# Keyteer/Mixed-precision_LU_Factorization

Hardware: AMD Instinct MI355X
Metric: LU GFLOP/s at N=32768 (1/2/4/8 GPUs); IR iterations to ||r||/||b||<1e-12 (higher is better)
Workload: dtype f64

## Files before the change

mixed-precision_lu_factorization_amd/csrc/factor_common.h:

```cpp
#pragma once
#include "mpf_internal.h"
#include <initializer_list>

struct FactorArgs {
    mpf_ctx *c; EvPool &ev; mpf_stats &st; const mpf_opts &o;
    double *d_A; int64_t lda, N; int32_t nb; int32_t *d_ipiv;
};
inline int pref_window_rows(const mpf_opts &o) { return o.trailing == MPF_TRAIL_FP64 ? HP_FP64_WINDOW_ROWS : 0; }
inline void stream_join(EvPool &ev, hipStream_t from, hipStream_t into) {
    hipEvent_t e = ev.get();
    hipEventRecord(e, from);
    hipStreamWaitEvent(into, e, 0);
}

int factor_check_args(mpf_ctx *c, const char *who, const char *ldname, int64_t N, int32_t nb, int64_t ld, const mpf_opts &o);
inline int wanted_superpanel(const mpf_ctx *c, const mpf_opts &o, int64_t N) {
    const bool f64 = o.trailing == MPF_TRAIL_FP64;
    int sb = f64 ? c->tune.superpanel_fp64 : c->tune.superpanel_fp16;
    if (!f64 && sb == 0) sb = (o.trailing == MPF_TRAIL_FP16 && N >= 24576) ? 6 : 4;
    return o.superpanel > 0 ? (o.superpanel > 8 ? 8 : o.superpanel) : sb;
}
int factor_report(mpf_ctx *c, mpf_stats &st, int rc, const std::function<hipError_t()> &wait, const char *what, const char *timeout_text);

struct PanelView {
    double *A; int64_t lda;
    int64_t k; int pr, pc;
    MovedList *ml; int32_t *ipiv;
};
int panel_pivots(const FactorArgs &f, const PanelView &v, hipStream_t s, int waiters, bool generic = false);
int panel_tail(const FactorArgs &f, const PanelView &v, hipStream_t s);
int panel_pieces(const FactorArgs &f, const PanelView &v, int np, const std::function<int(int)> &after_piece = nullptr);
int panel_chain(const FactorArgs &f, int64_t k, hipStream_t s);
struct ChainEnd { int rc = 0; hipEvent_t a = nullptr, b = nullptr; };
ChainEnd chain_behind(const FactorArgs &f, int64_t nx, hipEvent_t e1);
int factor_epilogue(const FactorArgs &f, int rc, bool sink, int sb, bool side_streams);

int launch_generic_update(mpf_ctx *c, const mpf_opts &o, int64_t m, int64_t n, int pc, const double *L21, int64_t ldl, double *U12, int64_t ldu);
inline int launch_inner_u_image(mpf_ctx *c, const mpf_opts &o, const double *U12, int64_t ldu, int pc, int64_t n, int64_t inner_u_off) {
    return launch_cvt_u12(c, U12, ldu, pc, n, o.trailing == MPF_TRAIL_FP16X3, inner_u_off);
}
inline int launch_inner_gemm(mpf_ctx *c, const mpf_opts &o, int64_t m, int64_t n, int pc, const double *L21, int64_t ldl, double *U12, int64_t ldu, int64_t inner_u_off) {
    if (o.trailing == MPF_TRAIL_FP64) return launch_dgemm_minus(c, m, n, pc, L21, ldl, U12, ldu, U12 + pc, ldu);
    return launch_hgemm_images(c, m, n, pc, U12 + pc, ldu, false, o.trailing == MPF_TRAIL_FP16X3, 0, 0, inner_u_off);
}

struct FarView {
    double *A; int64_t lda;
    float *W; int64_t ldw, ncols;
    const double *Lsp; int64_t ldl;
    const double *L11; int64_t ld11;
};
struct ImageGeom { int kst; int64_t inner_u_off, brow_l_off; };
inline ImageGeom image_geom(int64_t N, int64_t far_cap, int sb, int nb, int h_kmax, bool f64) {
    const int kst = (int)(((int64_t)sb * nb + 63) & ~(int64_t)63);
    return {kst, (!f64 && far_cap > 0) ? far_cap * kst : 0, N * h_kmax};
}
int far_zero_padding(const FactorArgs &f, int64_t ncols, const ImageGeom &g);
int far_block_row(const FactorArgs &f, const FarView &v, const ImageGeom &g, int64_t s0, int p);
int far_big_update(const FactorArgs &f, const FarView &v, const ImageGeom &g, int64_t s0, int64_t s1, int64_t col, int64_t ncols, int img);

struct RmView {
    double *A; int64_t lda;
    double *R; int64_t ldr;
    double *a(int64_t i, int64_t j) const { return A + j * lda + i; }
    double *r(int64_t i, int64_t j) const { return R + i * ldr + j; }
};
int rm_swap(const FactorArgs &f, const RmView &v, hipStream_t s, int64_t c, int64_t w, std::initializer_list<const MovedList *> lists, int64_t scratch_off);
int rm_solve_u(const FactorArgs &f, const RmView &v, hipStream_t s, const double *L11, int64_t ld11, int64_t k, int pc, int64_t c, int64_t w);
int rm_update(const FactorArgs &f, const RmView &v, hipStream_t s, int64_t ku, int K, int64_t r0, int64_t rows, int64_t c, int64_t w, const double *Limg, int64_t ldimg);
int rm_home(const FactorArgs &f, const RmView &v, hipStream_t s, int64_t row, int64_t rows, int64_t c, int64_t w, int64_t split = 0);
int rm_l_image(const FactorArgs &f, hipStream_t s, const double *src, int64_t lds, int64_t rows, int64_t cols, double *img, int64_t ldimg);
bool pivots_fit_beside_update(const mpf_ctx *c, int64_t rows);
int factor_lookahead_rm(mpf_ctx *c, double *d_A, int64_t lda, int64_t N, int32_t nb, int32_t *d_ipiv, const mpf_opts &o, mpf_stats &st, bool pairs);
```

mixed-precision_lu_factorization_amd/csrc/factor_rm.cpp:

```cpp
#include "factor_common.h"
#include <cstdio>

int rm_swap(const FactorArgs &f, const RmView &v, hipStream_t s, int64_t c, int64_t w, std::initializer_list<const MovedList *> lists, int64_t scratch_off) {
    return f.ev.timed(f.st.ms_laswp, s, [&] {
        int e = 0;
        for (const MovedList *ml : lists) if (!e) e = launch_laswp_from_list_rm64(f.c, v.r(0, c), v.ldr, w, ml, scratch_off);
        return e; });
}
int rm_solve_u(const FactorArgs &f, const RmView &v, hipStream_t s, const double *L11, int64_t ld11, int64_t k, int pc, int64_t c, int64_t w) {
    return f.ev.timed(f.st.ms_trsm, s, [&] { return launch_dtrsm_llnu_strided(f.c, pc, w, L11, ld11, v.r(k, c), v.ldr, 1); });
}
int rm_update(const FactorArgs &f, const RmView &v, hipStream_t s, int64_t ku, int K, int64_t r0, int64_t rows, int64_t c, int64_t w, const double *Limg, int64_t ldimg) {
    const int e = f.ev.timed(f.st.ms_gemm, s, [&] { return launch_dgemm_minus(f.c, w, rows, K, v.r(ku, c), v.ldr, Limg, ldimg, v.r(r0, c), v.ldr); });
    count_gemm(f.st, f.o, rows, w, K);
    return e;
}
int rm_home(const FactorArgs &f, const RmView &v, hipStream_t s, int64_t row, int64_t rows, int64_t c, int64_t w, int64_t split) {
    return f.ev.timed(f.st.ms_cvt, s, [&] {
        if (split <= 0) return launch_transpose64(f.c, v.a(row, c), v.lda, v.r(row, c), v.ldr, rows, w, false);
        int e = launch_transpose64(f.c, v.a(row, c), v.lda, v.r(row, c), v.ldr, split, w, false);
        if (!e) e = launch_transpose64(f.c, v.a(row + split, c), v.lda, v.r(row + split, c), v.ldr, rows - split, w, false);
        return e; });
}
int rm_l_image(const FactorArgs &f, hipStream_t s, const double *src, int64_t lds, int64_t rows, int64_t cols, double *img, int64_t ldimg) {
// ... 281 lines not shown
}

static int rm_turn_one_lane(const FactorArgs &f, const RmView &v, RmLoop &L, const RmTurn &t) {
    mpf_ctx *c = f.c; EvPool &ev = f.ev; hipStream_t S = c->stream, P = c->pstream, T = c->tstream;
    const int64_t N = f.N, k = t.k, nx = t.nx, n = t.n, ce = L.ce; const int pc = t.pc, pc2 = t.pc2;
    const double *L11 = v.a(k, k);
    const int64_t cw = ce - nx - pc2;
    int rc = 0;
    if (L.was_two) {
        stream_join(ev, T, S);
        if (L.chain_a) hipStreamWaitEvent(S, L.chain_a, 0);
        if (L.chain_b) hipStreamWaitEvent(S, L.chain_b, 0);
        L.was_two = false;
    }
    hipEvent_t lt_ready = ev.get();
    {
        stream_join(ev, S, P);
        StreamSwap sw(c, P);
        rc = rm_l_image(f, P, v.a(nx, k), v.lda, n, pc, t.LT, pc);
        hipEventRecord(lt_ready, P);
    }
    if (!rc) rc = rm_swap(f, v, S, nx, ce - nx, {t.lk}, 0);
    if (!rc) rc = rm_solve_u(f, v, S, L11, v.lda, k, pc, nx, t.ns);
    hipStreamWaitEvent(S, lt_ready, 0);
    if (!rc) rc = rm_update(f, v, S, k, pc, nx, n, nx, t.ns, t.LT, pc);
    if (rc) return rc;
    if (!t.has_next)
        return rm_home(f, v, S, k, N - k, nx, N - nx, pc);
    rc = rm_home(f, v, S, nx, N - nx, nx, pc2);
    if (rc) return rc;
    hipEvent_t e1 = ev.get();
    hipEventRecord(e1, S);
    const ChainEnd next = chain_behind(f, nx, e1);
    rc = next.rc;
    if (rc) return rc;
    if (cw > 0) rc = rm_solve_u(f, v, S, L11, v.lda, k, pc, nx + pc2, cw);
    if (rc) return rc;
    hipStream_t H = T ? T : S;
    {
        if (T) stream_join(ev, S, T);
        StreamSwap sw(c, H);
        rc = rm_home(f, v, H, k, pc, nx, ce - nx);
        if (L.sink && !rc && ce == N) sink_notify(c, (int)(k / f.nb) + 1, H);
    }
    if (!rc && cw > 0) rc = rm_update(f, v, S, k, pc, nx, n, nx + pc2, cw, t.LT, pc);
    if (rc) return rc;
    L.chain_a = next.a; L.chain_b = next.b;
    hipStreamWaitEvent(S, L.chain_a, 0);
    if (L.chain_b) hipStreamWaitEvent(S, L.chain_b, 0);
    if (f.o.verbose) printf("panel k=%lld rows=%lld cols=%d (look-ahead, row-major copy)\n", (long long)nx, (long long)(N - nx), pc2);
    return 0;
}

int factor_lookahead_rm(mpf_ctx *c, double *d_A, int64_t lda, int64_t N, int32_t nb, int32_t *d_ipiv, const mpf_opts &o, mpf_stats &st, bool pairs) {
    hipStream_t S = c->stream, P = c->pstream, T = c->tstream;
    EvPool ev(c);
    ev.keep = &st.ms_gemm;
    const FactorArgs f{c, ev, st, o, d_A, lda, N, nb, d_ipiv};
    const RmView v{d_A, lda, c->r64, N};
    int rc = 0;
    RmLoop L;
    L.sink = sink_take(c, d_A, lda, N, nb);
    L.lp = (c->late && !c->late->taken && c->late->nseg > 0 && lda == N) ? c->late : nullptr;
    if (L.lp) L.lp->taken = true;
    L.ce = L.lp ? L.lp->c0[0] : N;
    { hipEvent_t e = ev.get(); hipEventRecord(e, S); hipStreamWaitEvent(P, e, 0); if (T) hipStreamWaitEvent(T, e, 0); }
    const int pc0 = (int)(N < nb ? N : nb);
    if (N > 1) {
        hipEvent_t e0 = ev.get();
        {
            StreamSwap sw(c, P);
            rc = ev.timed(st.ms_hpanel, P, [&] {
                int e = launch_hgetf2(c, d_A, lda, nullptr, 0, (int)N, pc0, 0, d_ipiv, nullptr, 0, c->lists, 0, pref_window_rows(o));
                if (!e) e = launch_laswp_from_list(c, d_A, lda, pc0, c->lists);
                if (!e) e = launch_dgetf2_npv(c, d_A, lda, (int)N, pc0, o.fused_panel, 0);
                return e; });
            hipEventRecord(e0, P);
        }
        st.panels++;
        if (!rc && pc0 < L.ce) rc = rm_l_image(f, S, v.a(0, pc0), lda, N, L.ce - pc0, v.r(0, pc0), v.ldr);
        hipStreamWaitEvent(S, e0, 0);
        L.chain_a = e0;
    }
    L.init_done = ev.get();
    hipEventRecord(L.init_done, S);
    if (pairs && !rc && !L.sink && !L.lp && T && N > 1) rc = factor_rm_pairs(f, v, L);
    for (int64_t k = L.k0; k < N && rc == 0; k += nb) {
        const RmTurn t(f, k);
        if (N - k <= 1 || t.nx >= N) break;
        rc = rm_replay_late(f, v, L, t);
        if (rc) break;
        const int64_t cw = L.ce - t.nx - t.pc2;
        const bool want_two = T && c->tune.fp64_two_lanes > 0 && t.has_next && pivots_fit_beside_update(c, N - t.nx) &&
                              (N - t.nx) > c->tune.chain_pipeline_below && cw >= c->tune.fp64_two_lanes;
        if (!want_two) L.cm = -1;
        const bool resplit = want_two && lane_split(c, t.nx + t.pc2, L.ce, L.cm);
        if (L.cm >= 0) rc = rm_turn_two_lanes(f, v, L, t, resplit);
        else {
            rc = rm_turn_one_lane(f, v, L, t);
            if (!t.has_next) break;
        }
    }
    if (!rc && L.lp && L.lseg < L.lp->nseg) rc = fail(c, -1, "factor_lookahead_rm: a late column segment was never brought up to date (plan beyond the matrix)");
    if (T) stream_join(ev, T, S);
    stream_join(ev, P, S);
    return factor_epilogue(f, rc, L.sink, 1, true);
}
```

mixed-precision_lu_factorization_amd/csrc/laswp.hip:

```cpp
#include "mpf_internal.h"

constexpr int LASWP_CPB = 16;

__global__ __launch_bounds__(256) void laswp_plan_kernel(const int *ipiv, int k, int cols, MovedList *out) {
    __shared__ int slot[HP_MAXCOLS];
    __shared__ int rowof[2 * HP_MAXCOLS];
    __shared__ int content[2 * HP_MAXCOLS];
    __shared__ int used[2 * HP_MAXCOLS];
    __shared__ int count;
    const int t = threadIdx.x;
    for (int s = t; s < 2 * cols; s += 256) { content[s] = s; used[s] = s < cols; rowof[s] = s < cols ? k + s : -1; }
    if (t == 0) count = 0;
    __syncthreads();
    if (t < cols) {
        const int p = ipiv[t] - 1;
        int s;
        if (p < k + cols) s = p - k;
        else {
            int first = t;
            for (int i = 0; i < t; ++i)
                if (ipiv[i] - 1 == p) { first = i; break; }
            s = cols + first;
            if (first == t) { rowof[s] = p; used[s] = 1; }
        }
// ... 338 lines not shown
__global__ __launch_bounds__(256) void lazy_gather_kernel(const double *__restrict__ A, long long lda, long long n, long long r0,
                                                         int w, const int *__restrict__ G, long long g0, double *__restrict__ T, long long ldt) {
    const long long d = r0 + (long long)blockIdx.x * 256 + threadIdx.x;
    if (d >= n) return;
    const long long sr = G[d - g0];
    const int c0 = blockIdx.y * 16;
#pragma unroll 8
    for (int c = c0; c < c0 + 16 && c < w; ++c) T[(d - r0) + (long long)c * ldt] = A[sr + (long long)c * lda];
}
__global__ __launch_bounds__(256) void lazy_scatter_kernel(const double *__restrict__ A, long long lda, long long n, long long r0,
                                                          int w, const int *__restrict__ F, double *__restrict__ T, long long ldt) {
    const long long r = r0 + (long long)blockIdx.x * 256 + threadIdx.x;
    if (r >= n) return;
    const long long d = (long long)F[r] - r0;
    const int c0 = blockIdx.y * 16;
#pragma unroll 4
    for (int c = c0; c < c0 + 16 && c < w; ++c) T[d + (long long)c * ldt] = A[r + (long long)c * lda];
}
__global__ __launch_bounds__(256) void lazy_copyback_kernel(double *__restrict__ A, long long lda, long long n, long long r0, int w,
                                                           const double *__restrict__ T, long long ldt) {
    const long long r = r0 + (long long)blockIdx.x * 256 + threadIdx.x;
    if (r >= n) return;
    const int c0 = blockIdx.y * 16;
#pragma unroll 4
    for (int c = c0; c < c0 + 16 && c < w; ++c) A[r + (long long)c * lda] = T[(r - r0) + (long long)c * ldt];
}

constexpr int LAZY1_THREADS = 1024;
constexpr int LAZY1_SLOTS = 32;
__host__ __device__ inline long long lazy_snap_offset(long long n, long long step, long long q) {
    return (q - 1) * n - step * ((q - 1) * q / 2);
}
__global__ __launch_bounds__(LAZY1_THREADS) void lazy_map_all_kernel(int *F, int *G, long long n, int nb, int npanels, int sb,
                                                                    const MovedList *lists, int *snap) {
    const int t = threadIdx.x;
    for (long long i = t; i < n; i += LAZY1_THREADS) { F[i] = (int)i; G[i] = (int)i; }
    __syncthreads();
    for (int p = npanels - 1; p >= 1; --p) {
        const MovedList *ml = lists + p;
        int m = ml->n;
        if (m > LASWP_MAXMOVED) m = LASWP_MAXMOVED;
        int v = 0, s = 0;
        if (t < m) { v = F[ml->dst[t]]; s = ml->src[t]; }
        __syncthreads();
        if (t < m) { F[s] = v; G[v] = s; }
        __syncthreads();
        if (p % sb) continue;
        const long long r0 = (long long)p * nb;
        int *sq = snap + lazy_snap_offset(n, (long long)sb * nb, p / sb);
        for (long long d = r0 + t; d < n; d += LAZY1_THREADS) sq[d - r0] = G[d];
    }
}
constexpr int LAZY1_LDS_ROWS = 16384;
template <int SLOTS>
__global__ __launch_bounds__(LAZY1_THREADS) void lazy_apply_all_kernel(double *A, long long lda, long long n, int nb, int sb, int b0,
                                                                      const int *snap) {
    constexpr int H = SLOTS * LAZY1_THREADS < LAZY1_LDS_ROWS ? SLOTS * LAZY1_THREADS : LAZY1_LDS_ROWS;
    constexpr int PASSES = SLOTS * LAZY1_THREADS / H;
    __shared__ double seg[H];
    const int b = b0 + (int)(blockIdx.x / (unsigned)nb);
    const long long q = b / sb + 1;
    const long long r0 = q * sb * nb;
    const int rows = (int)(n - r0);
    const int *Gq = snap + lazy_snap_offset(n, (long long)sb * nb, q);
    double *col = A + ((long long)b * nb + (long long)(blockIdx.x % (unsigned)nb)) * lda + r0;
    const int t = threadIdx.x;
    double v[SLOTS];
    constexpr int GRP = SLOTS < 8 ? SLOTS : 8;
#pragma unroll
    for (int pass = 0; pass < PASSES; ++pass) {
        const int base = pass * H;
        if (pass > 0) __syncthreads();
#pragma unroll
        for (int j0 = 0; j0 < H / LAZY1_THREADS; j0 += GRP) {
            double x[GRP];
#pragma unroll
            for (int j = 0; j < GRP; ++j) {
                const int r = base + (j0 + j) * LAZY1_THREADS + t;
                x[j] = col[(unsigned)(r < rows ? r : rows - 1) & (unsigned)(SLOTS * LAZY1_THREADS - 1)];
            }
#pragma unroll
            for (int j = 0; j < GRP; ++j) seg[(j0 + j) * LAZY1_THREADS + t] = x[j];
            asm volatile("" ::: "memory");
        }
        __syncthreads();
#pragma unroll
        for (int i0 = 0; i0 < SLOTS; i0 += GRP) {
            int rel[GRP];
            double x[GRP];
#pragma unroll
            for (int i = 0; i < GRP; ++i) {
                const int d = (i0 + i) * LAZY1_THREADS + t;
                rel[i] = Gq[(unsigned)(d < rows ? d : rows - 1) & (unsigned)(SLOTS * LAZY1_THREADS - 1)] - (int)r0 - base;
            }
#pragma unroll
            for (int i = 0; i < GRP; ++i) {
                x[i] = seg[(unsigned)rel[i] < (unsigned)H ? rel[i] : 0];
                asm volatile("" : "+v"(x[i]));
            }
#pragma unroll
            for (int i = 0; i < GRP; ++i)
                if (PASSES == 1 || (unsigned)rel[i] < (unsigned)H) v[i0 + i] = x[i];
            asm volatile("" ::: "memory");
        }
    }
    __syncthreads();
#pragma unroll
    for (int i = 0; i < SLOTS; ++i) {
        const int d = i * LAZY1_THREADS + t;
        if (d < rows) col[(unsigned)d & (unsigned)(SLOTS * LAZY1_THREADS - 1)] = v[i];
    }
}
template <int SLOTS>
static void lazy_apply_launch(mpf_ctx *c, double *A, int64_t lda, int64_t N, int nb, int sb, int b0, int nblocks, const int *snap) {
    lazy_apply_all_kernel<SLOTS><<<(unsigned)((int64_t)nblocks * nb), LAZY1_THREADS, 0, c->stream>>>(A, lda, N, nb, sb, b0, snap);
}
int64_t lazy_snap_elems(int64_t N, int nb, int npanels, int sb) {
    if (sb < 1) sb = 1;
    return npanels < 2 ? 0 : lazy_snap_offset(N, (int64_t)sb * nb, (npanels - 1) / sb + 1);
}
static int launch_lazy_left_swaps_onepass(mpf_ctx *c, double *A, int64_t lda, int64_t N, int nb, int npanels, const MovedList *lists, int sb) {
    const int64_t step = (int64_t)sb * nb;
    const int Q = (npanels - 1) / sb;
    c->lazy_onepass_blocks = 0;
    if (Q < 1) return 0;
    const int64_t need = lazy_snap_elems(N, nb, npanels, sb);
    if (c->lazy_snap.cap() < need) {
        MPF_HIP_TRY(c, hipStreamSynchronize(c->stream));
        MPF_HIP_TRY(c, c->lazy_snap.grow(need));
    }
    int *snap = c->lazy_snap;
    lazy_map_all_kernel<<<1, LAZY1_THREADS, 0, c->stream>>>(c->Fmap, c->Fmap + N, N, nb, npanels, sb, lists, snap);
    int64_t cap = c->tune.lazy_onepass_max_rows;
    if (cap > (int64_t)LAZY1_THREADS * LAZY1_SLOTS) cap = (int64_t)LAZY1_THREADS * LAZY1_SLOTS;
    const int nblk = Q * sb;
    int b1 = nblk;
    for (int b = 0; b < nblk; ++b) {
        const int64_t q = b / sb + 1, r0 = q * step, rows = N - r0;
        if (rows <= cap) { b1 = b; break; }
        dim3 grid((unsigned)((rows + 255) / 256), (unsigned)((nb + 15) / 16));
        double *Ab = A + (int64_t)b * nb * lda;
        lazy_gather_kernel<<<grid, 256, 0, c->stream>>>(Ab, lda, N, r0, nb, snap + lazy_snap_offset(N, step, q), r0, c->perm_tmp, rows);
        lazy_copyback_kernel<<<grid, 256, 0, c->stream>>>(Ab, lda, N, r0, nb, c->perm_tmp, rows);
    }
    for (int b = b1; b < nblk;) {
        const int64_t rows = N - (b / sb + 1) * step;
        int slots = 2;
        while ((int64_t)LAZY1_THREADS * slots < rows) slots *= 2;
        int e = b + 1;
        while (e < nblk && (N - (e / sb + 1) * step) * 2 > (int64_t)LAZY1_THREADS * slots) ++e;
        if (slots == 2) e = nblk;
        switch (slots) {
        case 32: lazy_apply_launch<32>(c, A, lda, N, nb, sb, b, e - b, snap); break;
        case 16: lazy_apply_launch<16>(c, A, lda, N, nb, sb, b, e - b, snap); break;
        case 8: lazy_apply_launch<8>(c, A, lda, N, nb, sb, b, e - b, snap); break;
        case 4: lazy_apply_launch<4>(c, A, lda, N, nb, sb, b, e - b, snap); break;
        default: lazy_apply_launch<2>(c, A, lda, N, nb, sb, b, e - b, snap); break;
        }
        b = e;
    }
    c->lazy_onepass_blocks = nblk - b1;
    MPF_HIP_TRY(c, hipGetLastError());
    return 0;
// ... 31 lines not shown
```

mixed-precision_lu_factorization_amd/csrc/mpf_factor.cpp:

```cpp
#include "factor_common.h"
#include <climits>
#include <cstdio>

int factor_check_args(mpf_ctx *c, const char *who, const char *ldname, int64_t N, int32_t nb, int64_t ld, const mpf_opts &o) {
    const std::string w = std::string(who) + ": ";
    if (N <= 0 || nb <= 0) return fail(c, -1, w + "N and panel width must be positive");
    if (ld < N) return fail(c, -1, w + ldname + " < N");
    if (N > INT_MAX / 2) return fail(c, -1, w + "N too large");
    if (nb > 65535) return fail(c, -1, w + "panel width > 65535");
    if (o.trailing < MPF_TRAIL_FP64 || o.trailing > MPF_TRAIL_FP16X3) return fail(c, -1, w + "unknown trailing mode");
    return 0;
}

int factor_report(mpf_ctx *c, mpf_stats &st, int rc, const std::function<hipError_t()> &wait, const char *what, const char *timeout_text) {
    hipEventRecord(c->ev1, c->stream);
    const hipError_t se = wait();
    if (rc) return rc;
    if (se != hipSuccess) return fail(c, -2, std::string(what) + " failed: " + hipGetErrorString(se));
    float ms = 0;
    hipEventElapsedTime(&ms, c->ev0, c->ev1);
    st.ms_total = ms;
    int info = 0, flags0 = 0;
    MPF_HIP_TRY(c, hipMemcpy(&info, &c->ws->info, sizeof(int), hipMemcpyDeviceToHost));
    MPF_HIP_TRY(c, hipMemcpy(&flags0, &c->ws->hp_timeouts, sizeof(int), hipMemcpyDeviceToHost));
// ... 213 lines not shown
    return e;
}

ChainEnd chain_behind(const FactorArgs &f, int64_t nx, hipEvent_t e1) {
    mpf_ctx *c = f.c; EvPool &ev = f.ev;
    const PanelView v = panel_at(f, nx);
    hipStream_t P = c->pstream, T = c->tstream;
    const int np = dgetf2_npv_pieces(c, v.pc);
    const int waiters = (c->tune.gate_wait_value && c->hp_signal) ? 0 : laswp_gated_grid(v.pc);
    const bool piped = c->tune.chain_pipeline && np != 0 && T && P &&
        !(f.o.trailing == MPF_TRAIL_FP64 && v.pr > c->tune.chain_pipeline_below) &&
        hgetf2_fits_beside(c, v.pr, v.pc, waiters);
    ChainEnd r;
    hipStreamWaitEvent(P, e1, 0);
    if (!piped) {
        r.rc = panel_chain(f, nx, P);
        r.a = ev.get();
        hipEventRecord(r.a, P);
        return r;
    }
    hipStreamWaitEvent(T, e1, 0);
    {
        StreamSwap sw(c, P);
        r.rc = panel_pivots(f, v, P, waiters);
        r.a = ev.get();
        hipEventRecord(r.a, P);
    }
    if (!r.rc) {
        StreamSwap sw(c, T);
        r.rc = ev.timed(f.st.ms_dpanel, T, [&] { return panel_pieces(f, v, np); });
        r.b = ev.get();
        hipEventRecord(r.b, T);
    }
    f.st.panels++;
    return r;
}

int factor_epilogue(const FactorArgs &f, int rc, bool sink, int sb, bool side_streams) {
    mpf_ctx *c = f.c;
    hipStream_t S = c->stream;
    const int npanels = (int)((f.N + f.nb - 1) / f.nb);
    if (sink) sink_notify(c, npanels, S);
    else if (!rc) {
        rc = f.ev.timed(f.st.ms_laswp, S, [&] { return launch_lazy_left_swaps(c, f.d_A, f.lda, f.N, f.nb, npanels, c->lists, sb); });
        f.st.lazy_onepass_blocks = c->lazy_onepass_blocks;
    }
    hipError_t se = sink_stream_wait(c, S);
    hipError_t sp = side_streams ? sink_stream_wait(c, c->pstream) : hipSuccess;
    if (side_streams && c->tstream) { const hipError_t stt = sink_stream_wait(c, c->tstream); if (sp == hipSuccess) sp = stt; }
    if (!rc && (se != hipSuccess || sp != hipSuccess))
        return fail(c, -2, std::string("factorization failed: ") + hipGetErrorString(se != hipSuccess ? se : sp));
    f.ev.collect();
    f.st.lookahead = side_streams ? 1 : 0;
    return rc;
}

static int factor_lookahead(mpf_ctx *c, double *d_A, int64_t lda, int64_t N, int32_t nb, int32_t *d_ipiv,
                            const mpf_opts &o, mpf_stats &st) {
    hipStream_t S = c->stream, P = c->pstream;
    EvPool ev(c);
    ev.keep = &st.ms_gemm;
    const FactorArgs f{c, ev, st, o, d_A, lda, N, nb, d_ipiv};
    int rc = 0;
    const bool sink = sink_take(c, d_A, lda, N, nb);
    stream_join(ev, S, P);
    {
        const int pc = (int)(N < nb ? N : nb), pr = (int)N;
        if (pr > 1) {
            rc = ev.timed(st.ms_hpanel, S, [&] {
                int e = launch_hgetf2(c, d_A, lda, nullptr, 0, pr, pc, 0, d_ipiv, nullptr, 0, c->lists, 0, pref_window_rows(o));
                const int64_t first = (int64_t)pc + nb < N ? (int64_t)pc + nb : N;
                if (!e) e = launch_laswp_from_list(c, d_A, lda, first, c->lists);
                if (!e) e = launch_dgetf2_npv(c, d_A, lda, pr, pc, o.fused_panel, 0);
                return e;
            });
            st.panels++;
        }
    }
    for (int64_t k = 0; k < N && rc == 0; k += nb) {
        const int pc = (int)((N - k) < nb ? (N - k) : nb);
        if (N - k <= 1 || k + pc >= N) break;
        const int64_t n = N - k - pc;
        const int64_t nx = k + pc;
        const int pc2 = (int)((N - nx) < nb ? (N - nx) : nb);
        const bool has_next = (N - nx) > 1;
        double *Ap = d_A + k * lda + k;
        double *A12 = d_A + nx * lda + k;
        const int64_t ns = has_next ? pc2 : n;
        rc = ev.timed(st.ms_trsm, S, [&] { return launch_dtrsm_llnu(c, pc, ns, Ap, lda, A12, lda); });
        if (rc) break;
        rc = ev.timed(st.ms_gemm, S, [&] {
            int e = o.trailing != MPF_TRAIL_FP64 ? launch_cvt_l21(c, Ap + pc, lda, n, pc, o.trailing == MPF_TRAIL_FP16X3) : 0;
            if (!e) e = trail_gemm(c, o, n, ns, pc, Ap + pc, A12, A12 + pc, lda);
            return e; });
        if (rc) break;
        count_gemm(st, o, n, ns, pc);
        if (!has_next) break;
        hipEvent_t e1 = ev.get();
        hipEventRecord(e1, S);
        const ChainEnd next = chain_behind(f, nx, e1);
        rc = next.rc;
        if (rc) break;
        if (n > pc2) {
            rc = ev.timed(st.ms_laswp, S, [&] {
                return launch_laswp_from_list(c, d_A + (nx + pc2) * lda, lda, N - nx - pc2, c->lists + (k / nb)); });
            if (rc) break;
            double *A12r = A12 + (int64_t)pc2 * lda;
            rc = ev.timed(st.ms_trsm, S, [&] { return launch_dtrsm_llnu(c, pc, n - pc2, Ap, lda, A12r, lda); });
            if (rc) break;
            if (sink) sink_notify(c, (int)(k / nb) + 1, S);
            rc = ev.timed(st.ms_gemm, S, [&] { return trail_gemm(c, o, n, n - pc2, pc, Ap + pc, A12r, A12r + pc, lda); });
            if (rc) break;
            count_gemm(st, o, n, n - pc2, pc);
        }
        hipStreamWaitEvent(S, next.a, 0);
        if (next.b) hipStreamWaitEvent(S, next.b, 0);
        rc = ev.timed(st.ms_laswp, S, [&] {
            const int64_t s0 = nx + pc2;
            const int64_t sw = (N - s0) < nb ? (N - s0) : nb;
            return sw > 0 ? launch_laswp_from_list(c, d_A + s0 * lda, lda, sw, c->lists + (nx / nb)) : 0;
        });
        if (o.verbose) printf("panel k=%lld rows=%lld cols=%d (look-ahead)\n", (long long)nx, (long long)(N - nx), pc2);
    }
    if (sink) stream_join(ev, P, S);
    return factor_epilogue(f, rc, sink, 1, true);
}

static int factor_superpanel(mpf_ctx *c, double *d_A, int64_t lda, int64_t N, int32_t nb, int32_t *d_ipiv, const mpf_opts &o,
                             mpf_stats &st, int sb, bool overlap) {
    hipStream_t S = c->stream, P = overlap ? c->pstream : c->stream;
    hipStream_t Ci = (overlap && c->tstream) ? c->tstream : c->stream;
    const bool lanes = Ci != S;
    EvPool ev(c);
    ev.keep = &st.ms_gemm;
    const FactorArgs f{c, ev, st, o, d_A, lda, N, nb, d_ipiv};
    int rc = 0;
    const bool split = o.trailing == MPF_TRAIL_FP16X3;
    const bool f64 = o.trailing == MPF_TRAIL_FP64;
    const bool use32 = !f64 && c->tune.fp16_work32 != 0 && N > (int64_t)(sb + 1) * nb;
    float *W = nullptr;
    const int64_t ldw = N;
    if (use32) {
        MPF_HIP_TRY(c, c->w32.grow(N * N));
        W = c->w32;
    }
    if (overlap) stream_join(ev, S, P);
    const int64_t sbw = (int64_t)sb * nb;
    const ImageGeom g = image_geom(N, N - (int64_t)(sb + 1) * nb, sb, nb, c->h_kmax, f64);
    auto width = [&](int64_t k) { return (int)((N - k) < nb ? (N - k) : nb); };
    auto side_chain = [&](int64_t kx, hipEvent_t e1, hipEvent_t &e2) -> int {
        if (!overlap) return panel_chain(f, kx, S);
        const ChainEnd next = chain_behind(f, kx, e1);
        e2 = next.a;
        if (!next.rc && next.b) {
            e2 = ev.get();
            hipStreamWaitEvent(c->tstream, next.a, 0);
            hipEventRecord(e2, c->tstream);
        }
        return next.rc;
    };
    hipEvent_t img_ready = nullptr;
    auto l21_image = [&](int64_t k, int pc) -> int {
        if (f64) return 0;
        const int64_t mrows = N - k - pc;
        if (mrows <= 0) return 0;
        hipStream_t Is = (lanes && P != S) ? P : Ci;
        if (Is != Ci) stream_join(ev, Ci, Is);
        StreamSwap sw(c, Is);
        int e = ev.timed(st.ms_cvt, Is, [&] { return launch_cvt_l21(c, d_A + k * lda + k + pc, lda, mrows, pc, split); });
        if (Is != Ci) { img_ready = ev.get(); hipEventRecord(img_ready, Is); } else img_ready = nullptr;
        return e;
    };
    auto inner_step = [&](int64_t k, int pc, int64_t col0, int64_t ncols, bool first) -> int {
        if (ncols <= 0) return 0;
        StreamSwap sw(c, Ci);
        double *Ap = d_A + k * lda + k, *A12 = d_A + col0 * lda + k;
// ... 167 lines not shown
```

mixed-precision_lu_factorization_amd/csrc/mpf_host.cpp:

```cpp
#include "mpf_internal.h"
#include <climits>
#include <cstdio>
#include <cstdlib>
#include <cstring>

std::string &noctx_error() { static thread_local std::string s; return s; }

namespace {
struct OptDesc { const char *name, *env; size_t off; bool wide; long long lo, hi; };
#define OPT_I(field, env, lo, hi) {#field, env, offsetof(MpfTuning, field), false, lo, hi}
#define OPT_L(field, env, lo, hi) {#field, env, offsetof(MpfTuning, field), true, lo, hi}
const OptDesc kOpts[] = {
    OPT_I(safe_pivots, "MPF_SAFE_PIVOTS", 0, 1),
    OPT_I(pivot_fp64, "MPF_PIVOT_FP64", 0, 2),
    OPT_I(chain_pipeline, "MPF_CHAIN_PIPELINE", 0, 1),
    OPT_L(chain_pipeline_below, "MPF_CHAIN_PIPELINE_BELOW", 0, 1ll << 40),
    OPT_I(fp16_work32, "MPF_FP16_WORK32", 0, 1),
    OPT_I(superpanel_fp16, "MPF_SUPERPANEL", 0, 8),
    OPT_I(superpanel_fp64, "MPF_SUPERPANEL_FP64", 1, 8),
    OPT_I(no_lookahead, "MPF_NO_LOOKAHEAD", 0, 1),
    OPT_I(verbose, "MPF_VERBOSE", 0, 1),
    OPT_I(timeline, "MPF_TIMELINE", 0, 1),
    OPT_L(hp_spin_limit, "MPF_HP_SPIN_LIMIT", 1, 1ll << 31),
    OPT_L(hp_gate_ticks, "MPF_HP_GATE_TICKS", 0, 1ll << 40),
    OPT_I(hp_acq_fence, "MPF_HP_ACQ_FENCE", 0, 1),
    OPT_I(hp_window, "MPF_HP_WINDOW", -1, 1 << 30),
    OPT_I(hgemm_pad, "MPF_HGEMM_PAD", 0, 65536),
    OPT_I(hgemm_split_pad, "MPF_HGEMM_SPLIT_PAD", 0, 65536),
    OPT_I(hgemm_big, "MPF_HGEMM_BIG", 0, 1),
    OPT_I(hgemm_big_tile, "MPF_HGEMM_BIG_TILE", 0, 5),
    OPT_I(hgemm_mfma16, "MPF_HGEMM_MFMA16", 0, 1),
    OPT_I(dgemm_dma, "MPF_DGEMM_DMA", 0, 1),
    OPT_I(lazy_gather, "MPF_LAZY_GATHER", 0, 2),
    OPT_I(lazy_onepass_max_rows, "MPF_LAZY_ONEPASS_MAX_ROWS", 0, 32768),
    OPT_I(dpanel_fused_form, "MPF_DPANEL_FUSED", 0, 1),
    OPT_I(dist_instalments, "MPF_DIST_INSTALMENTS", 0, 1),
    OPT_L(dist_instalment_min_bytes, "MPF_DIST_INSTALMENT_MIN_BYTES", 0, 1ll << 40),
    OPT_I(generic_fused, "MPF_GENERIC_FUSED", 0, 1),
    OPT_I(fp16_fused, "MPF_FP16_FUSED", 0, 1),
    OPT_I(fp64_rowmajor, "MPF_FP64_ROWMAJOR", 0, 1),
    OPT_L(fp64_rowmajor_min_n, "MPF_FP64_ROWMAJOR_MIN_N", 0, 1ll << 40),
    OPT_I(trsm_laswp_fused, "MPF_TRSM_LASWP_FUSED", 0, 1),
    OPT_I(fp64_two_lanes, "MPF_FP64_TWO_LANES", 0, 1 << 30),
    OPT_I(fp64_lane_a_pct, "MPF_FP64_LANE_A_PCT", 20, 90),
    OPT_I(fp64_pair, "MPF_FP64_PAIR", 0, 1),
    OPT_L(fp64_pair_min_n, "MPF_FP64_PAIR_MIN_N", 0, 1ll << 40),
    OPT_I(event_timers, "MPF_EVENT_TIMERS", 0, 2),
    OPT_I(dist_world1_loop, "MPF_DIST_WORLD1_LOOP", 0, 1),
    OPT_I(gesv_fp64_tflops, "MPF_GESV_FP64_TFLOPS", 0, 1000),
    OPT_I(gate_wait_value, "MPF_GATE_WAIT_VALUE", 0, 1),
    OPT_I(host_sink, "MPF_HOST_SINK", 0, 1),
    OPT_I(sink_trace, "MPF_SINK_TRACE", 0, 1),
    OPT_I(hp_half_slabs, "MPF_HP_HALF_SLABS", 0, 1),
    OPT_I(hp_half_slabs_rows, "MPF_HP_HALF_SLABS_ROWS", 256, 32768),
    OPT_I(hp_local_xcd, "MPF_HP_LOCAL_XCD", 0, 2),
    OPT_I(host_late_parts, "MPF_HOST_LATE_PARTS", 0, 4),
    OPT_L(host_late_min_n, "MPF_HOST_LATE_MIN_N", 0, 1ll << 40),
    OPT_I(host_first_pct, "MPF_HOST_FIRST_PCT", 5, 100),
    OPT_I(host_late_q_pct, "MPF_HOST_LATE_Q_PCT", 1, 1000),
    OPT_L(host_sink_min_n, "MPF_HOST_SINK_MIN_N", 0, 1ll << 40),
    OPT_I(dist_solve_p2p, "MPF_DIST_SOLVE_P2P", 0, 1),
    OPT_I(gmres_group_tiles, "MPF_GMRES_GROUP_TILES", 0, 16),
#ifdef MPF_PROBE
    OPT_I(hp_stamp, "MPF_HP_STAMP", 0, 1),
    OPT_I(hp_r256_upto, "MPF_HP_R256_UPTO", 0, 1 << 30),
    OPT_I(dgemm_w8, "MPF_DGEMM_W8", 0, 1),
    OPT_I(gemm_lds_pad, "MPF_GEMM_LDS_PAD", 0, 65536),
    OPT_I(hgemm_big_reg, "MPF_HGEMM_BIG_REG", 0, 1),
    OPT_I(hgemm_dbg, "MPF_HGEMM_DBG", 0, 8191),
#endif
};
#undef OPT_I
#undef OPT_L
void opt_store(MpfTuning &t, const OptDesc &d, long long v) {
    if (v < d.lo) v = d.lo;
    if (v > d.hi) v = d.hi;
    char *p = (char *)&t + d.off;
    if (d.wide) *(long long *)p = v; else *(int *)p = (int)v;
}
long long opt_load(const MpfTuning &t, const OptDesc &d) {
    const char *p = (const char *)&t + d.off;
    return d.wide ? *(const long long *)p : (long long)*(const int *)p;
}
void tuning_from_env(MpfTuning &t) {
    for (const OptDesc &d : kOpts)
        if (const char *e = getenv(d.env)) if (*e) opt_store(t, d, atoll(e));
}
}

extern "C" {

int mpf_create(mpf_ctx **out, int device) {
    if (!out) return -1;
    *out = nullptr;
// ... 295 lines not shown
```

mixed-precision_lu_factorization_amd/csrc/mpf_internal.h:

```cpp
#pragma once
#include <hip/hip_runtime.h>
#include <stdint.h>
#include <string>
#include <vector>
#include <functional>
#include "../../include/mpf_c.h"

constexpr int HP_R = 256;
constexpr int HP_T = 512;
constexpr int HP_MAXG = 256;
constexpr int HP_MAXCOLS = 256;
constexpr int LASWP_MAXMOVED = 2 * HP_MAXCOLS;

struct MovedList {
    int n;
    int pad[3];
    int src[LASWP_MAXMOVED];
    int dst[LASWP_MAXMOVED];
};

struct MpfWorkspace {
    unsigned long long cand[2][HP_MAXG];
    int flags[16];
    unsigned long long rowbuf[2][HP_MAXG][HP_MAXCOLS / 2];
    int hp_timeouts;
    int pad0[3];
    MovedList list0;
    int info;
    int pad[3];
    unsigned long long hp_stamps[8];
    unsigned long long hp_progress;
    unsigned long long hp_xcd_target;
    unsigned long long hp_xcd_roles;
};

struct MpfTuning {
    int safe_pivots = 0;
    int pivot_fp64 = 0;
    int chain_pipeline = 1;
    long long chain_pipeline_below = 10240;
    int fp16_work32 = 1;
    int superpanel_fp16 = 0;
    int superpanel_fp64 = 1;
    int no_lookahead = 0;
    int verbose = 0;
    int timeline = 0;
    long long hp_spin_limit = 1ll << 21;
    long long hp_gate_ticks = 200000000ll;
    int hp_window = -1;
    int hp_acq_fence = 0;
    int hgemm_pad = 0;
    int hgemm_split_pad = 32768;
    int hgemm_big = 1;
    int hgemm_mfma16 = 1;
    int hgemm_big_tile = 0;
    int dgemm_dma = 1;
    int lazy_gather = 2;
    int lazy_onepass_max_rows = 32768;
    int dpanel_fused_form = 1;
    int dist_instalments = 1;
    long long dist_instalment_min_bytes = 8ll << 20;
    int fp16_fused = 0;
    int generic_fused = 1;
    int fp64_rowmajor = 1;
    long long fp64_rowmajor_min_n = 8192;
    int trsm_laswp_fused = 1;
    int fp64_two_lanes = 8192;
    int dist_solve_p2p = 0;
    int host_sink = 1;
    int hp_local_xcd = 1;
    int hp_half_slabs = 1;
    int hp_half_slabs_rows = 16384;
    int sink_trace = 0;
    int host_late_parts = 3;
    long long host_late_min_n = 16384;
    int host_first_pct = 25;
    int host_late_q_pct = 110;
    long long host_sink_min_n = 4096;
    int gate_wait_value = 0;
    int gesv_fp64_tflops = 0;
    int dist_world1_loop = 0;
    int event_timers = 1;
    int fp64_lane_a_pct = 50;
    int fp64_pair = 1;
    long long fp64_pair_min_n = 16384;
    int gmres_group_tiles = 0;
#ifdef MPF_PROBE
    int hp_stamp = 0;
    int hp_r256_upto = 1 << 30;
    int dgemm_w8 = 1;
    int gemm_lds_pad = 0;
    int hgemm_dbg = 0;
    int hgemm_big_reg = 0;
#endif
};

template <class T, bool Pinned = false>
struct Buf {
    Buf() = default;
    Buf(const Buf &) = delete;
    Buf &operator=(const Buf &) = delete;
    ~Buf() { release(); }
    hipError_t grow(int64_t n) {
        if (n <= cap_) return hipSuccess;
        release();
        void *q = nullptr;
        const hipError_t e = Pinned ? hipHostMalloc(&q, (size_t)n * sizeof(T)) : hipMalloc(&q, (size_t)n * sizeof(T));
        if (e != hipSuccess) return e;
        p_ = (T *)q;
        cap_ = n;
        return hipSuccess;
    }
    void release() {
        if (p_) (void)(Pinned ? hipHostFree(p_) : hipFree(p_));
        p_ = nullptr;
        cap_ = 0;
    }
    T *get() const { return p_; }
// ... 331 lines not shown
```

Baseline: 55210.

## Add optional in-place tail hand-over for row-major FP64 LU and tweak lazy gather codegen

Adds a tunable threshold (default 0, disabled) at which the row-major FP64 look-ahead loop copies the remaining row-major trailing matrix back to column-major home layout and finishes with the in-place column-major look-ahead turns. The column-major look-ahead loop body is factored into a reusable lookahead_turn function. Separately, the lazy_apply_all_kernel for 32 slots gets compiler barriers that re-materialise the thread index and regroup the writeback loop, aiming to reduce register pressure or improve scheduling. The tail path is off by default, so only the kernel codegen tweak affects default runs.

```diff
diff --git a/mixed-precision_lu_factorization_amd/csrc/factor_common.h b/mixed-precision_lu_factorization_amd/csrc/factor_common.h
--- a/mixed-precision_lu_factorization_amd/csrc/factor_common.h
+++ b/mixed-precision_lu_factorization_amd/csrc/factor_common.h
@@ -34,6 +34,7 @@
 struct ChainEnd { int rc = 0; hipEvent_t a = nullptr, b = nullptr; };
 ChainEnd chain_behind(const FactorArgs &f, int64_t nx, hipEvent_t e1);
 int factor_epilogue(const FactorArgs &f, int rc, bool sink, int sb, bool side_streams);
+int lookahead_turn(const FactorArgs &f, int64_t k, bool sink, hipEvent_t &chain_a, hipEvent_t &chain_b, bool &more);
 
 int launch_generic_update(mpf_ctx *c, const mpf_opts &o, int64_t m, int64_t n, int pc, const double *L21, int64_t ldl, double *U12, int64_t ldu);
 inline int launch_inner_u_image(mpf_ctx *c, const mpf_opts &o, const double *U12, int64_t ldu, int pc, int64_t n, int64_t inner_u_off) {
diff --git a/mixed-precision_lu_factorization_amd/csrc/factor_rm.cpp b/mixed-precision_lu_factorization_amd/csrc/factor_rm.cpp
--- a/mixed-precision_lu_factorization_amd/csrc/factor_rm.cpp
+++ b/mixed-precision_lu_factorization_amd/csrc/factor_rm.cpp
@@ -357,6 +357,18 @@
     return 0;
 }
 
+static int rm_hand_over(const FactorArgs &f, const RmView &v, RmLoop &L, const RmTurn &t) {
+    mpf_ctx *c = f.c; EvPool &ev = f.ev; hipStream_t S = c->stream, T = c->tstream;
+    if (T) stream_join(ev, T, S);
+    if (L.chain_a) hipStreamWaitEvent(S, L.chain_a, 0);
+    if (L.chain_b) hipStreamWaitEvent(S, L.chain_b, 0);
+    L.was_two = false;
+    int rc = rm_home(f, v, S, t.k, f.N - t.k, t.nx, f.N - t.nx);
+    if (!rc) rc = ev.timed(f.st.ms_laswp, S, [&] { return launch_laswp_from_list(c, v.a(0, t.nx), v.lda, t.ns, t.lk); });
+    if (f.o.verbose) printf("panel k=%lld rows=%lld (row-major copy: %lld x %lld home, in place from here)\n", (long long)t.k, (long long)(f.N - t.k), (long long)(f.N - t.k), (long long)(f.N - t.nx));
+    return rc;
+}
+
 int factor_lookahead_rm(mpf_ctx *c, double *d_A, int64_t lda, int64_t N, int32_t nb, int32_t *d_ipiv, const mpf_opts &o, mpf_stats &st, bool pairs) {
     hipStream_t S = c->stream, P = c->pstream, T = c->tstream;
     EvPool ev(c);
@@ -390,9 +402,16 @@
     L.init_done = ev.get();
     hipEventRecord(L.init_done, S);
     if (pairs && !rc && !L.sink && !L.lp && T && N > 1) rc = factor_rm_pairs(f, v, L);
+    const int64_t tail_n = (L.sink || L.lp) ? 0 : c->tune.fp64_tail_inplace_n;
     for (int64_t k = L.k0; k < N && rc == 0; k += nb) {
         const RmTurn t(f, k);
         if (N - k <= 1 || t.nx >= N) break;
+        if (N - k <= tail_n) {
+            rc = rm_hand_over(f, v, L, t);
+            bool more = true;
+            for (; k < N && rc == 0 && more; k += nb) rc = lookahead_turn(f, k, false, L.chain_a, L.chain_b, more);
+            break;
+        }
         rc = rm_replay_late(f, v, L, t);
         if (rc) break;
         const int64_t cw = L.ce - t.nx - t.pc2;
diff --git a/mixed-precision_lu_factorization_amd/csrc/laswp.hip b/mixed-precision_lu_factorization_amd/csrc/laswp.hip
--- a/mixed-precision_lu_factorization_amd/csrc/laswp.hip
+++ b/mixed-precision_lu_factorization_amd/csrc/laswp.hip
@@ -414,6 +414,10 @@
     }
 }
 constexpr int LAZY1_LDS_ROWS = 16384;
+template <int SLOTS> __device__ __forceinline__ int lazy_fresh_tid(int t) {
+    if (SLOTS == 32) asm volatile("" : "+v"(t));
+    return t;
+}
 template <int SLOTS>
 __global__ __launch_bounds__(LAZY1_THREADS) void lazy_apply_all_kernel(double *A, long long lda, long long n, int nb, int sb, int b0,
                                                                       const int *snap) {
@@ -436,13 +440,14 @@
 #pragma unroll
         for (int j0 = 0; j0 < H / LAZY1_THREADS; j0 += GRP) {
             double x[GRP];
+            const int tl = lazy_fresh_tid<SLOTS>(t);
 #pragma unroll
             for (int j = 0; j < GRP; ++j) {
-                const int r = base + (j0 + j) * LAZY1_THREADS + t;
+                const int r = base + (j0 + j) * LAZY1_THREADS + tl;
                 x[j] = col[(unsigned)(r < rows ? r : rows - 1) & (unsigned)(SLOTS * LAZY1_THREADS - 1)];
             }
 #pragma unroll
-            for (int j = 0; j < GRP; ++j) seg[(j0 + j) * LAZY1_THREADS + t] = x[j];
+            for (int j = 0; j < GRP; ++j) seg[(j0 + j) * LAZY1_THREADS + tl] = x[j];
             asm volatile("" ::: "memory");
         }
         __syncthreads();
@@ -450,27 +455,38 @@
         for (int i0 = 0; i0 < SLOTS; i0 += GRP) {
             int rel[GRP];
             double x[GRP];
+            const int tl = lazy_fresh_tid<SLOTS>(t);
 #pragma unroll
             for (int i = 0; i < GRP; ++i) {
-                const int d = (i0 + i) * LAZY1_THREADS + t;
+                const int d = (i0 + i) * LAZY1_THREADS + tl;
                 rel[i] = Gq[(unsigned)(d < rows ? d : rows - 1) & (unsigned)(SLOTS * LAZY1_THREADS - 1)] - (int)r0 - base;
             }
 #pragma unroll
             for (int i = 0; i < GRP; ++i) {
                 x[i] = seg[(unsigned)rel[i] < (unsigned)H ? rel[i] : 0];
-                asm volatile("" : "+v"(x[i]));
+                if (SLOTS != 32) asm volatile("" : "+v"(x[i]));
             }
-#pragma unroll
-            for (int i = 0; i < GRP; ++i)
+            if (SLOTS == 32) {
+#pragma unroll
+                for (int i = 0; i < GRP; ++i) asm volatile("" : "+v"(x[i]));
+            }
+#pragma unroll
+            for (int i = 0; i < GRP; ++i) {
                 if (PASSES == 1 || (unsigned)rel[i] < (unsigned)H) v[i0 + i] = x[i];
+                if (pass > 0) asm volatile("" : "+v"(v[i0 + i]));
+            }
             asm volatile("" ::: "memory");
         }
     }
     __syncthreads();
 #pragma unroll
-    for (int i = 0; i < SLOTS; ++i) {
-        const int d = i * LAZY1_THREADS + t;
-        if (d < rows) col[(unsigned)d & (unsigned)(SLOTS * LAZY1_THREADS - 1)] = v[i];
+    for (int i0 = 0; i0 < SLOTS; i0 += GRP) {
+        const int tl = lazy_fresh_tid<SLOTS>(t);
+#pragma unroll
+        for (int i = i0; i < i0 + GRP; ++i) {
+            const int d = i * LAZY1_THREADS + tl;
+            if (d < rows) col[(unsigned)d & (unsigned)(SLOTS * LAZY1_THREADS - 1)] = v[i];
+        }
     }
 }
 template <int SLOTS>
diff --git a/mixed-precision_lu_factorization_amd/csrc/mpf_factor.cpp b/mixed-precision_lu_factorization_amd/csrc/mpf_factor.cpp
--- a/mixed-precision_lu_factorization_amd/csrc/mpf_factor.cpp
+++ b/mixed-precision_lu_factorization_amd/csrc/mpf_factor.cpp
@@ -289,6 +289,60 @@
         return fail(c, -2, std::string("factorization failed: ") + hipGetErrorString(se != hipSuccess ? se : sp));
     f.ev.collect();
     f.st.lookahead = side_streams ? 1 : 0;
+    return rc;
+}
+
+int lookahead_turn(const FactorArgs &f, int64_t k, bool sink, hipEvent_t &chain_a, hipEvent_t &chain_b, bool &more) {
+    mpf_ctx *c = f.c; EvPool &ev = f.ev; mpf_stats &st = f.st; const mpf_opts &o = f.o;
+    hipStream_t S = c->stream;
+    double *d_A = f.d_A; const int64_t lda = f.lda, N = f.N; const int32_t nb = f.nb;
+    int rc = 0;
+    more = false;
+    const int pc = (int)((N - k) < nb ? (N - k) : nb);
+    if (N - k <= 1 || k + pc >= N) return 0;
+    const int64_t n = N - k - pc;
+    const int64_t nx = k + pc;
+    const int pc2 = (int)((N - nx) < nb ? (N - nx) : nb);
+    const bool has_next = (N - nx) > 1;
+    double *Ap = d_A + k * lda + k;
+    double *A12 = d_A + nx * lda + k;
+    const int64_t ns = has_next ? pc2 : n;
+    rc = ev.timed(st.ms_trsm, S, [&] { return launch_dtrsm_llnu(c, pc, ns, Ap, lda, A12, lda); });
+    if (rc) return rc;
+    rc = ev.timed(st.ms_gemm, S, [&] {
+        int e = o.trailing != MPF_TRAIL_FP64 ? launch_cvt_l21(c, Ap + pc, lda, n, pc, o.trailing == MPF_TRAIL_FP16X3) : 0;
+        if (!e) e = trail_gemm(c, o, n, ns, pc, Ap + pc, A12, A12 + pc, lda);
+        return e; });
+    if (rc) return rc;
+    count_gemm(st, o, n, ns, pc);
+    if (!has_next) return 0;
+    hipEvent_t e1 = ev.get();
+    hipEventRecord(e1, S);
+    const ChainEnd next = chain_behind(f, nx, e1);
+    rc = next.rc;
+    if (rc) return rc;
+    if (n > pc2) {
+        rc = ev.timed(st.ms_laswp, S, [&] {
+            return launch_laswp_from_list(c, d_A + (nx + pc2) * lda, lda, N - nx - pc2, c->lists + (k / nb)); });
+        if (rc) return rc;
+        double *A12r = A12 + (int64_t)pc2 * lda;
+        rc = ev.timed(st.ms_trsm, S, [&] { return launch_dtrsm_llnu(c, pc, n - pc2, Ap, lda, A12r, lda); });
+        if (rc) return rc;
+        if (sink) sink_notify(c, (int)(k / nb) + 1, S);
+        rc = ev.timed(st.ms_gemm, S, [&] { return trail_gemm(c, o, n, n - pc2, pc, Ap + pc, A12r, A12r + pc, lda); });
+        if (rc) return rc;
+        count_gemm(st, o, n, n - pc2, pc);
+    }
+    chain_a = next.a; chain_b = next.b;
+    hipStreamWaitEvent(S, chain_a, 0);
+    if (chain_b) hipStreamWaitEvent(S, chain_b, 0);
+    rc = ev.timed(st.ms_laswp, S, [&] {
+        const int64_t s0 = nx + pc2;
+        const int64_t sw = (N - s0) < nb ? (N - s0) : nb;
+        return sw > 0 ? launch_laswp_from_list(c, d_A + s0 * lda, lda, sw, c->lists + (nx / nb)) : 0;
+    });
+    if (o.verbose) printf("panel k=%lld rows=%lld cols=%d (look-ahead)\n", (long long)nx, (long long)(N - nx), pc2);
+    more = rc == 0;
     return rc;
 }
 
@@ -314,51 +368,9 @@
             st.panels++;
         }
     }
-    for (int64_t k = 0; k < N && rc == 0; k += nb) {
-        const int pc = (int)((N - k) < nb ? (N - k) : nb);
-        if (N - k <= 1 || k + pc >= N) break;
-        const int64_t n = N - k - pc;
-        const int64_t nx = k + pc;
-        const int pc2 = (int)((N - nx) < nb ? (N - nx) : nb);
-        const bool has_next = (N - nx) > 1;
-        double *Ap = d_A + k * lda + k;
-        double *A12 = d_A + nx * lda + k;
-        const int64_t ns = has_next ? pc2 : n;
-        rc = ev.timed(st.ms_trsm, S, [&] { return launch_dtrsm_llnu(c, pc, ns, Ap, lda, A12, lda); });
-        if (rc) break;
-        rc = ev.timed(st.ms_gemm, S, [&] {
-            int e = o.trailing != MPF_TRAIL_FP64 ? launch_cvt_l21(c, Ap + pc, lda, n, pc, o.trailing == MPF_TRAIL_FP16X3) : 0;
-            if (!e) e = trail_gemm(c, o, n, ns, pc, Ap + pc, A12, A12 + pc, lda);
-            return e; });
-        if (rc) break;
-        count_gemm(st, o, n, ns, pc);
-        if (!has_next) break;
-        hipEvent_t e1 = ev.get();
-        hipEventRecord(e1, S);
-        const ChainEnd next = chain_behind(f, nx, e1);
-        rc = next.rc;
-        if (rc) break;
-        if (n > pc2) {
-            rc = ev.timed(st.ms_laswp, S, [&] {
-                return launch_laswp_from_list(c, d_A + (nx + pc2) * lda, lda, N - nx - pc2, c->lists + (k / nb)); });
-            if (rc) break;
-            double *A12r = A12 + (int64_t)pc2 * lda;
-            rc = ev.timed(st.ms_trsm, S, [&] { return launch_dtrsm_llnu(c, pc, n - pc2, Ap, lda, A12r, lda); });
-            if (rc) break;
-            if (sink) sink_notify(c, (int)(k / nb) + 1, S);
-            rc = ev.timed(st.ms_gemm, S, [&] { return trail_gemm(c, o, n, n - pc2, pc, Ap + pc, A12r, A12r + pc, lda); });
-            if (rc) break;
-            count_gemm(st, o, n, n - pc2, pc);
-        }
-        hipStreamWaitEvent(S, next.a, 0);
-        if (next.b) hipStreamWaitEvent(S, next.b, 0);
-        rc = ev.timed(st.ms_laswp, S, [&] {
-            const int64_t s0 = nx + pc2;
-            const int64_t sw = (N - s0) < nb ? (N - s0) : nb;
-            return sw > 0 ? launch_laswp_from_list(c, d_A + s0 * lda, lda, sw, c->lists + (nx / nb)) : 0;
-        });
-        if (o.verbose) printf("panel k=%lld rows=%lld cols=%d (look-ahead)\n", (long long)nx, (long long)(N - nx), pc2);
-    }
+    hipEvent_t chain_a = nullptr, chain_b = nullptr;
+    bool more = true;
+    for (int64_t k = 0; k < N && rc == 0 && more; k += nb) rc = lookahead_turn(f, k, sink, chain_a, chain_b, more);
     if (sink) stream_join(ev, P, S);
     return factor_epilogue(f, rc, sink, 1, true);
 }
diff --git a/mixed-precision_lu_factorization_amd/csrc/mpf_host.cpp b/mixed-precision_lu_factorization_amd/csrc/mpf_host.cpp
--- a/mixed-precision_lu_factorization_amd/csrc/mpf_host.cpp
+++ b/mixed-precision_lu_factorization_amd/csrc/mpf_host.cpp
@@ -40,6 +40,7 @@
     OPT_I(fp16_fused, "MPF_FP16_FUSED", 0, 1),
     OPT_I(fp64_rowmajor, "MPF_FP64_ROWMAJOR", 0, 1),
     OPT_L(fp64_rowmajor_min_n, "MPF_FP64_ROWMAJOR_MIN_N", 0, 1ll << 40),
+    OPT_L(fp64_tail_inplace_n, "MPF_FP64_TAIL_INPLACE_N", 0, 1ll << 40),
     OPT_I(trsm_laswp_fused, "MPF_TRSM_LASWP_FUSED", 0, 1),
     OPT_I(fp64_two_lanes, "MPF_FP64_TWO_LANES", 0, 1 << 30),
     OPT_I(fp64_lane_a_pct, "MPF_FP64_LANE_A_PCT", 20, 90),
diff --git a/mixed-precision_lu_factorization_amd/csrc/mpf_internal.h b/mixed-precision_lu_factorization_amd/csrc/mpf_internal.h
--- a/mixed-precision_lu_factorization_amd/csrc/mpf_internal.h
+++ b/mixed-precision_lu_factorization_amd/csrc/mpf_internal.h
@@ -64,6 +64,7 @@
     int generic_fused = 1;
     int fp64_rowmajor = 1;
     long long fp64_rowmajor_min_n = 8192;
+    long long fp64_tail_inplace_n = 0;
     int trsm_laswp_fused = 1;
     int fp64_two_lanes = 8192;
     int dist_solve_p2p = 0;
```

Result: no change. 55330 (median of 6 runs) (+0.2%).
